# facebookresearch/hyperreel

Hardware: NVIDIA H100
Metric: Mrays/s at 65k-ray x 32-sample batch (higher is better)
Workload: dtype f32 (sample net bf16x3 split on wgmma, fp32 accumulate)

## Files before the change

hyperreel_b200/csrc/hr_mlp_tc2.cu:

```cuda
#include <cuda.h>
#include <cuda_bf16.h>

#include <cstdio>
#include <cstdlib>
#include <cstring>

#include "hr_encode.cuh"
#include "hr_handle.h"
#include "hr_tc_prims.cuh"

namespace hr {

namespace tc2 {
using namespace tc;

constexpr int NSTAGE = 4;
constexpr int STAGE_BYTES = 8192;
constexpr int KSTEP_BYTES = 4096;
constexpr int CONSUMERS = 2;
constexpr int NTHREADS = (CONSUMERS + 1) * 128;
constexpr int PRODUCER_REGS = 40;
constexpr int CONSUMER_REGS = 232;
static_assert(128 * PRODUCER_REGS + CONSUMERS * 128 * CONSUMER_REGS <= 65536, "register file");

constexpr int A_BYTES = 16 * KSTEP_BYTES;
constexpr int OFF_AHI = 0;
constexpr int OFF_ALO = OFF_AHI + A_BYTES;
constexpr int X_BYTES = 4 * KSTEP_BYTES;
constexpr int OFF_X = OFF_ALO + A_BYTES;
constexpr int OFF_B = OFF_X + 2 * X_BYTES;
constexpr int OFF_BAR = OFF_B + CONSUMERS * NSTAGE * STAGE_BYTES;
constexpr int SMEM_BYTES = OFF_BAR + 128;
static_assert(SMEM_BYTES <= 232448, "shared memory budget");

constexpr int BAR_FULL = 0;
constexpr int BAR_EMPTY = BAR_FULL + CONSUMERS * NSTAGE;
static_assert((BAR_EMPTY + CONSUMERS * NSTAGE) * 8 <= 128, "barrier block");

constexpr int NB_RET = 3;
constexpr int NB_WR = 5;
constexpr int NB_XW = 7;
constexpr int NB_XR = 9;

}

template <int W, bool SAVE, bool NARROW>
__global__ void __launch_bounds__(tc2::NTHREADS, 1)
mlp_tc2_kernel(const __grid_constant__ hr_config cfg, const __grid_constant__ MlpTcPack pk, const float* __restrict__ rays,
               float* __restrict__ heads, long long n_rays, float* __restrict__ rays_copy, const TrainSave sv) {
  using namespace tc2;
  constexpr int WH = W / 2;
  constexpr int NACC = WH / 2;
  constexpr int NK = W / 16;
  constexpr int NKH = NK / 2;
  constexpr int IMG_BYTES = WH * 64;
  constexpr int KPS = STAGE_BYTES / IMG_BYTES;
  static_assert(KPS * IMG_BYTES == STAGE_BYTES && NKH % KPS == 0 && NK * KSTEP_BYTES <= A_BYTES, "pass width");
  extern __shared__ __align__(128) uint8_t smem[];
  const uint32_t sbase = smem_u32(smem);
  const int tid = threadIdx.x, warp = tid >> 5, lane = tid & 31;
  auto bar = [&](int slot) -> uint32_t { return sbase + OFF_BAR + slot * 8; };

  {
    const char* w = reinterpret_cast<const char*>(pk.wpack);
    const long long lines = pk.wpack_bytes >> 7;
    for (long long i = (long long)blockIdx.x * NTHREADS + tid; i < lines; i += (long long)gridDim.x * NTHREADS)
      asm volatile("prefetch.global.L2 [%0];" ::"l"(w + i * 128));
  }
  for (int i = tid; i < (2 * X_BYTES) / 16; i += NTHREADS)
    reinterpret_cast<uint4*>(smem + OFF_X)[i] = make_uint4(0u, 0u, 0u, 0u);
  if (tid == 0) {
    for (int s = 0; s < CONSUMERS * NSTAGE; ++s) { mbar_init(bar(BAR_FULL + s), 1); mbar_init(bar(BAR_EMPTY + s), 1); }
    asm volatile("fence.mbarrier_init.release.cluster;" ::: "memory");
  }
  __syncthreads();

  const long long n_tiles = (n_rays + BM - 1) / BM;
  const int n_passes = pk.n_passes;
  const long long n_iters = ((long long)blockIdx.x < n_tiles) ? (n_tiles - 1 - blockIdx.x) / gridDim.x + 1 : 0;

  if (warp >= CONSUMERS * 4) {
    setmaxnreg_dec<PRODUCER_REGS>();
    const int g = warp - CONSUMERS * 4;
    if (g < CONSUMERS && lane == 0) {
      const long long half_bytes = pk.wpack_bytes / CONSUMERS;
      const int n_stages = (int)(half_bytes / STAGE_BYTES);
      const uint32_t full0 = bar(BAR_FULL + g * NSTAGE), empty0 = bar(BAR_EMPTY + g * NSTAGE);
      const uint32_t ring = sbase + OFF_B + (uint32_t)(g * NSTAGE * STAGE_BYTES);
      uint32_t stage = 0, phase = 0;
      for (long long iter = 0; iter < n_iters; ++iter) {
        const uint8_t* src = reinterpret_cast<const uint8_t*>(pk.wpack) + g * half_bytes;
        for (int i = 0; i < n_stages; ++i) {
          mbar_wait(empty0 + stage * 8, phase ^ 1);
          mbar_expect_tx(full0 + stage * 8, STAGE_BYTES);
          bulk_g2s(ring + stage * STAGE_BYTES, src, STAGE_BYTES, full0 + stage * 8);
          src += STAGE_BYTES;
          if (++stage == NSTAGE) { stage = 0; phase ^= 1; }
        }
      }
    }
    return;
  }

  setmaxnreg_inc<CONSUMER_REGS>();
  const int wg = warp >> 2;
  const int wt = tid & 127;
  const int rowq = (warp & 3) * 16 + (lane >> 2);
  const int q2 = (lane & 3) * 2;
  const int col0 = wg * WH;
  const int in_chunks = pk.in_chunks;
  const int L = cfg.mlp_layers;
  const uint32_t x_lo_off = (uint32_t)(2 * in_chunks * KSTEP_BYTES);
  const uint32_t full0 = bar(BAR_FULL + wg * NSTAGE), empty0 = bar(BAR_EMPTY + wg * NSTAGE);
  const uint32_t ring = sbase + OFF_B + (uint32_t)(wg * NSTAGE * STAGE_BYTES);
  const bool vec_ok = ((reinterpret_cast<uintptr_t>(rays) | reinterpret_cast<uintptr_t>(rays_copy)) & 15) == 0;
  int x_last = 0;
  for (int p = 0; p < n_passes; ++p)
    if (pk.passes[p].first_chunk == 0) x_last = p;
  uint32_t stage = 0, phase = 0;
  int pend = -1;

  float acc[2][NACC];

  auto stage_begin = [&]() {
    mbar_wait(full0 + stage * 8, phase);
    wgmma_fence();
    acc_fence(acc[0]);
    acc_fence(acc[1]);
  };
  auto stage_end = [&]() {
    wgmma_commit();
    acc_fence(acc[0]);
    acc_fence(acc[1]);
    wgmma_wait<1>();
    if (pend >= 0 && wt == 0) mbar_arrive(empty0 + pend * 8);
    pend = (int)stage;
    if (++stage == NSTAGE) { stage = 0; phase ^= 1; }
  };
  auto b_img = [&](int sub) -> uint32_t { return ring + stage * STAGE_BYTES + (uint32_t)sub * IMG_BYTES; };
  auto kstep = [&](uint32_t a, uint32_t a_lo, uint32_t b, uint32_t scale) {
    const uint64_t bh = gmma_desc(b, WH * 16, 128), bl = gmma_desc(b + WH * 32, WH * 16, 128);
    const uint64_t ah0 = gmma_desc(a, 2048, 128), ah1 = gmma_desc(a + 1024, 2048, 128);
    const uint64_t al0 = gmma_desc(a + a_lo, 2048, 128), al1 = gmma_desc(a + a_lo + 1024, 2048, 128);
    wgmma_ss(acc[0], ah0, bh, scale);
    wgmma_ss(acc[1], ah1, bh, scale);
    wgmma_ss(acc[0], al0, bh, 1u);
    wgmma_ss(acc[1], al1, bh, 1u);
    wgmma_ss(acc[0], ah0, bl, 1u);
    wgmma_ss(acc[1], ah1, bl, 1u);
  };
  auto run_pass = [&](const TcPass& P, bool fresh, bool x_ret, bool ret) {
    int ki = 0;
    if (P.first_chunk == 0) {
      for (; ki < 2 * in_chunks; ki += KPS) {
        stage_begin();
#pragma unroll
        for (int sub = 0; sub < KPS; ++sub)
          kstep(sbase + OFF_X + (uint32_t)(ki + sub) * KSTEP_BYTES, x_lo_off, b_img(sub), (ki + sub) != 0 ? 1u : 0u);
        stage_end();
      }
    }
    if (P.first_chunk + P.n_chunks > in_chunks) {
      const uint32_t scale0 = ki != 0 ? 1u : 0u;
#pragma unroll
      for (int kk = 0; kk < NK; ++kk) {
        if (kk % KPS == 0) {
          if (fresh && kk == (wg == 0 ? NKH : 0)) {
            if (wg == 0) pair_arrive(NB_WR + 0);
            pair_wait(NB_WR + (wg ^ 1));
          }
          stage_begin();
        }
        kstep(sbase + OFF_AHI + (uint32_t)kk * KSTEP_BYTES, OFF_ALO - OFF_AHI, b_img(kk % KPS), kk != 0 ? 1u : scale0);
        if (kk % KPS == KPS - 1) {
          stage_end();
          if (x_ret && kk == KPS - 1) pair_arrive(NB_XR + wg);
          if (ret && wg == 1 && kk == NKH + KPS - 1) pair_arrive(NB_RET + 1);
        }
      }
    }
  };
  auto drain = [&]() {
    wgmma_wait<0>();
    acc_fence(acc[0]);
    acc_fence(acc[1]);
    if (pend >= 0 && wt == 0) mbar_arrive(empty0 + pend * 8);
    pend = -1;
  };
  const int st_row = (warp & 3) * 16 + 8 * ((lane >> 3) & 1) + (lane & 7);
  const uint32_t st_off = ks_slot(st_row, lane >> 4);
  auto store_hidden = [&](const float* bias, int layer, long long tile) {
#pragma unroll
    for (int kk = 0; kk < NKH; ++kk) {
      float2 b[2];
#pragma unroll
      for (int jj = 0; jj < 2; ++jj) b[jj] = __ldg(reinterpret_cast<const float2*>(bias + col0 + 8 * (2 * kk + jj) + q2));
#pragma unroll
      for (int m = 0; m < 2; ++m) {
        uint32_t hi[4], lo[4];
#pragma unroll
        for (int jj = 0; jj < 2; ++jj) {
          const int j = 2 * kk + jj, k = col0 + 8 * j + q2;
#pragma unroll
          for (int h = 0; h < 2; ++h) {
            float t0 = acc[m][4 * j + 2 * h] + b[jj].x, t1 = acc[m][4 * j + 2 * h + 1] + b[jj].y;
            t0 = fmaxf(t0, t0 * cfg.leaky_slope);
            t1 = fmaxf(t1, t1 * cfg.leaky_slope);
            split2(t0, t1, hi[2 * jj + h], lo[2 * jj + h]);
            if constexpr (SAVE) {
              const long long ray = tile * BM + 64 * m + rowq + 8 * h;
              if (ray < n_rays) *reinterpret_cast<float2*>(sv.act + layer * sv.act_stride + ray * W + k) = make_float2(t0, t1);
            }
          }
        }
        const uint32_t a = sbase + st_off + (uint32_t)m * 1024u + (uint32_t)(wg * NKH + kk) * KSTEP_BYTES;
        stmatrix_x4(a + OFF_AHI, hi);
        stmatrix_x4(a + OFF_ALO, lo);
      }
    }
  };
  auto encode = [&](long long tile, bool after_x) {
    if (after_x) pair_wait(NB_XR + (wg ^ 1));
    const int r = wg * 64 + (wt & 63), part = wt >> 6;
    const long long ray = tile * BM + r;
    auto put = [&](int k, float val) {
      if constexpr (SAVE) {
        if (ray < n_rays) sv.enc[ray * sv.ld_enc + k] = val;
      }
      const __nv_bfloat16 hi = __float2bfloat16_rn(val);
      const __nv_bfloat16 lo = __float2bfloat16_rn(val - __bfloat162float(hi));
      const uint32_t off = (uint32_t)(k >> 4) * KSTEP_BYTES + ks_slot(r, (k >> 3) & 1) + (uint32_t)(k & 7) * 2u;
      *reinterpret_cast<__nv_bfloat16*>(smem + OFF_X + off) = hi;
      *reinterpret_cast<__nv_bfloat16*>(smem + OFF_X + x_lo_off + off) = lo;
    };
    if (ray < n_rays) {
      float rbuf[16];
      const float* src = rays + ray * cfg.c_in;
      if (cfg.c_in == 8 && vec_ok) {
        const float4 a = *reinterpret_cast<const float4*>(src), b = *reinterpret_cast<const float4*>(src + 4);
        rbuf[0] = a.x; rbuf[1] = a.y; rbuf[2] = a.z; rbuf[3] = a.w; rbuf[4] = b.x; rbuf[5] = b.y; rbuf[6] = b.z; rbuf[7] = b.w;
        if (rays_copy != nullptr && part == 0) {
          float4* dst = reinterpret_cast<float4*>(rays_copy + ray * 8);
          dst[0] = a; dst[1] = b;
        }
      } else {
        for (int i = 0; i < cfg.c_in; ++i) rbuf[i] = src[i];
        if (rays_copy != nullptr && part == 0)
          for (int i = 0; i < cfg.c_in; ++i) rays_copy[ray * cfg.c_in + i] = rbuf[i];
      }
      encode_ray_features(cfg, rbuf, part, 2, put);
      if constexpr (SAVE) {
        if (part == 0)
          for (int k = cfg.mlp_in; k < sv.ld_enc; ++k) sv.enc[ray * sv.ld_enc + k] = 0.0f;
      }
    } else if (part == 0) {
      for (int k = 0; k < cfg.mlp_in; ++k) put(k, 0.0f);
    }
    fence_async_smem();
    wg_sync(1 + wg);
    pair_arrive(NB_XW + wg);
  };

  for (long long iter = 0; iter < n_iters; ++iter) {
    const long long tile = iter * gridDim.x + blockIdx.x;
    const bool more = iter + 1 < n_iters;
    if (iter == 0) encode(tile, false);
    pair_wait(NB_XW + (wg ^ 1));
    for (int p = 0; p < n_passes; ++p) {
      const TcPass& P = pk.passes[p];
      const bool reads_a = P.first_chunk + P.n_chunks > in_chunks;
      const bool hidden = p < L - 1;
      const bool ret = reads_a && (hidden || (p == n_passes - 1 && more));
      const bool x_ret = p == x_last && more;
      run_pass(P, reads_a && P.wait_a != 0, x_ret, ret);
      drain();
      if (x_ret && !reads_a) pair_arrive(NB_XR + wg);
      if (ret && wg == 0) pair_arrive(NB_RET + 0);
      if (hidden) {
        wg_sync(1 + wg);
        if (p > 0 || iter > 0) pair_wait(NB_RET + (wg ^ 1));
        store_hidden(pk.bias + P.bias_off, p, tile);
        fence_async_smem();
        wg_sync(1 + wg);
        if (wg == 1) pair_arrive(NB_WR + 1);
      } else {
        const float* bias = pk.bias + P.bias_off;
        if constexpr (SAVE) {
#pragma unroll
          for (int m = 0; m < 2; ++m)
#pragma unroll
            for (int h = 0; h < 2; ++h) {
              const long long ray = tile * BM + 64 * m + rowq + 8 * h;
              if (ray >= n_rays) continue;
              float* row = heads + ray * cfg.mlp_out;
#pragma unroll
              for (int j = 0; j < WH / 8; ++j) {
                const int c = col0 + 8 * j + q2;
                if (P.out_col0 + c < cfg.mlp_out) {
                  const float2 b = __ldg(reinterpret_cast<const float2*>(bias + c));
                  const int c0 = P.out_col0 + c, c1 = c0 + 1, S = cfg.n_samples;
                  row[(c0 % S) * cfg.head_stride + c0 / S] = acc[m][4 * j + 2 * h] + b.x;
                  if (c1 < cfg.mlp_out) row[(c1 % S) * cfg.head_stride + c1 / S] = acc[m][4 * j + 2 * h + 1] + b.y;
                }
              }
            }
        } else if constexpr (NARROW) {
          const bool pairs = (cfg.mlp_out % 2) == 0 && (reinterpret_cast<uintptr_t>(heads) & 7) == 0;
#pragma unroll
          for (int j = 0; j < WH / 8; ++j) {
            const int c = col0 + 8 * j + q2, c0 = P.out_col0 + c;
            const float2 b = __ldg(reinterpret_cast<const float2*>(bias + c));
#pragma unroll
            for (int m = 0; m < 2; ++m)
#pragma unroll
              for (int h = 0; h < 2; ++h) {
                const long long ray = tile * BM + 64 * m + rowq + 8 * h;
                if (ray >= n_rays || c0 >= cfg.mlp_out) continue;
                float* dst = heads + ray * cfg.mlp_out + c0;
                const float v0 = acc[m][4 * j + 2 * h] + b.x, v1 = acc[m][4 * j + 2 * h + 1] + b.y;
                if (pairs) {
                  *reinterpret_cast<float2*>(dst) = make_float2(v0, v1);
                } else {
                  dst[0] = v0;
                  if (c0 + 1 < cfg.mlp_out) dst[1] = v1;
                }
              }
          }
        } else {
          const bool odd = (lane & 1) != 0;
#pragma unroll
          for (int jp = 0; jp < WH / 16; ++jp) {
            const int j = 2 * jp, c = col0 + 8 * j + q2;
            const float2 b0 = __ldg(reinterpret_cast<const float2*>(bias + c));
            const float2 b1 = __ldg(reinterpret_cast<const float2*>(bias + c + 8));
#pragma unroll
            for (int m = 0; m < 2; ++m)
#pragma unroll
              for (int h = 0; h < 2; ++h) {
                const float2 v0 = make_float2(acc[m][4 * j + 2 * h] + b0.x, acc[m][4 * j + 2 * h + 1] + b0.y);
                const float2 v1 = make_float2(acc[m][4 * j + 4 + 2 * h] + b1.x, acc[m][4 * j + 4 + 2 * h + 1] + b1.y);
                const float2 send = odd ? v0 : v1;
                const float2 recv = make_float2(__shfl_xor_sync(0xffffffffu, send.x, 1), __shfl_xor_sync(0xffffffffu, send.y, 1));
                const int c4 = odd ? c + 6 : c;
                const long long ray = tile * BM + 64 * m + rowq + 8 * h;
                if (ray < n_rays && P.out_col0 + c4 < cfg.mlp_out)
                  *reinterpret_cast<float4*>(heads + ray * cfg.mlp_out + P.out_col0 + c4) =
                      odd ? make_float4(recv.x, recv.y, v1.x, v1.y) : make_float4(v0.x, v0.y, recv.x, recv.y);
              }
          }
        }
      }
      if (x_ret) encode(tile + gridDim.x, true);
    }
  }
}

int pack_mlp_tc2(SampleNet& net, const float* const* w_dev, const float* const* b_dev, cudaStream_t st) {
  const hr_config& c = net.cfg;
  MlpTcPack& pk = net.tc;
  size_t& alloc_bytes = net.tc_alloc_bytes;
  int& alloc_bias = net.tc_alloc_bias;
  const int W = c.mlp_width;
  if (W != 128 && W != 256) return hr_fail("tensor-core sample net: hidden width must be 128 or 256 (got %d)", W);
  if (c.mlp_in > 64) return hr_fail("tensor-core sample net: encoded input wider than 64 features (%d)", c.mlp_in);
  const int in_chunks = (c.mlp_in + 31) / 32;
  const int L = c.mlp_layers;
  MlpTcPack np_{};
  np_.in_chunks = in_chunks;
  int np = 0, bias_off = 0;
  size_t bytes = 0;
  for (int l = 0; l < L; ++l) {
    const bool last = (l == L - 1);
    const int out = last ? c.mlp_out : W;
    const int n_parts = (out + W - 1) / W;
    for (int part = 0; part < n_parts; ++part) {
      if (np >= HR_TC_MAX_PASSES) return hr_fail("tensor-core sample net: too many passes (%d output columns)", c.mlp_out);
      TcPass& P = np_.passes[np++];
      const bool reads_input = (l == 0 || l == c.mlp_skip);
      P.layer = l;
      P.n = W;
      P.first_chunk = reads_input ? 0 : in_chunks;
      P.n_chunks = (l == 0) ? in_chunks : (W / 32 + (reads_input ? in_chunks : 0));
      P.bias_off = bias_off;
      P.is_final = last ? 1 : 0;
      P.out_col0 = part * W;
      P.wait_a = (part == 0) ? 1 : 0;
      bias_off += P.n;
      bytes += (size_t)P.n_chunks * 2 * P.n * 64;
    }
  }
  np_.n_passes = np;
  np_.bias_count = bias_off;
  np_.wpack_bytes = (long long)bytes;
  if (alloc_bytes != bytes || alloc_bias != bias_off || !pk.wpack) {
    if (pk.wpack) cudaFree(const_cast<void*>(pk.wpack));
    if (pk.bias) cudaFree(const_cast<float*>(pk.bias));
    pk.wpack = nullptr; pk.bias = nullptr;
    alloc_bytes = 0; alloc_bias = 0;
    void* wp = nullptr; float* bp = nullptr;
    cudaError_t e = cudaMalloc(&wp, bytes);
    if (e != cudaSuccess) return hr_fail("cudaMalloc(tc weights %zu): %s", bytes, cudaGetErrorString(e));
    e = cudaMalloc((void**)&bp, (size_t)bias_off * sizeof(float));
    if (e != cudaSuccess) { cudaFree(wp); return hr_fail("cudaMalloc(tc bias): %s", cudaGetErrorString(e)); }
    np_.wpack = wp; np_.bias = bp;
    alloc_bytes = bytes; alloc_bias = bias_off;
    for (int narrow = 0; narrow < 2 && e == cudaSuccess; ++narrow) {
      auto kern = (W == 256) ? (narrow ? mlp_tc2_kernel<256, false, true> : mlp_tc2_kernel<256, false, false>)
                             : (narrow ? mlp_tc2_kernel<128, false, true> : mlp_tc2_kernel<128, false, false>);
      e = cudaFuncSetAttribute(kern, cudaFuncAttributeMaxDynamicSharedMemorySize, tc2::SMEM_BYTES);
    }
    if (e != cudaSuccess) return hr_fail("cudaFuncSetAttribute(mlp_tc2_kernel): %s", cudaGetErrorString(e));
  } else {
    np_.wpack = pk.wpack; np_.bias = pk.bias;
  }
  pk = np_;
  uint8_t* wp = (uint8_t*)const_cast<void*>(pk.wpack);
  float* bp = const_cast<float*>(pk.bias);
  const int WH = W / 2;
  for (int half = 0; half < 2; ++half) {
    size_t off = (size_t)half * (bytes / 2);
    for (int p = 0; p < np; ++p) {
      const TcPass& P = pk.passes[p];
      const int l = P.layer;
      const bool last = (l == L - 1), skip = (l == c.mlp_skip), first = (l == 0);
      const int in_src = first ? c.mlp_in : (skip ? c.mlp_in + W : W);
      launch_pack_tc_pass(w_dev[l], b_dev[l], wp + off, bp + P.bias_off + half * WH, WH, P.first_chunk, P.n_chunks, in_src,
                          c.mlp_in, skip ? 1 : 0, in_chunks, last ? c.mlp_out : W, last ? c.n_samples : 0, c.head_stride,
                          P.out_col0 + half * WH, st);
      off += (size_t)P.n_chunks * 2 * WH * 64;
    }
  }
  cudaError_t e = cudaGetLastError();
  if (e != cudaSuccess) return hr_fail("tc pack launch failed: %s", cudaGetErrorString(e));
  return 0;
}

void free_mlp_tc2(SampleNet& net) {
  if (net.tc.wpack) cudaFree(const_cast<void*>(net.tc.wpack));
  if (net.tc.bias) cudaFree(const_cast<float*>(net.tc.bias));
  net.tc.wpack = nullptr; net.tc.bias = nullptr;
  net.tc_alloc_bytes = 0; net.tc_alloc_bias = 0;
}

cudaError_t launch_mlp_tc2(const hr_config& cfg, const MlpTcPack& pk, const float* rays, float* heads, long long n, int num_sms,
                           cudaStream_t stream, float* rays_copy) {
  long long tiles = (n + tc::BM - 1) / tc::BM;
  int grid = (int)(tiles < num_sms ? tiles : num_sms);
  if (grid < 1) grid = 1;
  const bool narrow = (cfg.mlp_out % 4) != 0 || ((uintptr_t)heads % 16) != 0;
  auto kern = cfg.mlp_width == 256 ? (narrow ? mlp_tc2_kernel<256, false, true> : mlp_tc2_kernel<256, false, false>)
                                   : (narrow ? mlp_tc2_kernel<128, false, true> : mlp_tc2_kernel<128, false, false>);
  if (cfg.mlp_width != 256 && cfg.mlp_width != 128) return cudaErrorInvalidValue;
  kern<<<grid, tc2::NTHREADS, tc2::SMEM_BYTES, stream>>>(cfg, pk, rays, heads, n, rays_copy, TrainSave{});
  return cudaGetLastError();
}

cudaError_t launch_mlp_tc2_train(const hr_config& cfg, const MlpTcPack& pk, const float* rays, float* heads, long long n,
                                 int num_sms, cudaStream_t stream, const TrainSave& sv) {
  long long tiles = (n + tc::BM - 1) / tc::BM;
  int grid = (int)(tiles < num_sms ? tiles : num_sms);
  if (grid < 1) grid = 1;
  auto kern = cfg.mlp_width == 256 ? mlp_tc2_kernel<256, true, false> : mlp_tc2_kernel<128, true, false>;
  if (cfg.mlp_width != 256 && cfg.mlp_width != 128) return cudaErrorInvalidValue;
  cudaError_t e = cudaFuncSetAttribute(kern, cudaFuncAttributeMaxDynamicSharedMemorySize, tc2::SMEM_BYTES);
  if (e != cudaSuccess) return e;
  kern<<<grid, tc2::NTHREADS, tc2::SMEM_BYTES, stream>>>(cfg, pk, rays, heads, n, nullptr, sv);
  return cudaGetLastError();
}

}
```

Baseline: 156.9.

## Move next-tile ray encoding to producer-warpgroup encoder warps with mbarrier handoff

Encoding of the next tile's input features moves off the consumer warpgroups and onto the two idle warps of the producer warpgroup. These warps fill the X buffer, which is double-buffered when the input fits in one chunk, and hand it over through full/empty mbarriers. This replaces the named-barrier handshake and the inline encode that consumers ran after each tile. Consumer registers drop from 232 to 224 to give the producer warpgroup 56, which risks spills in the consumer accumulator path, and only 64 threads now encode each tile.

```diff
diff --git a/hyperreel_b200/csrc/hr_mlp_tc2.cu b/hyperreel_b200/csrc/hr_mlp_tc2.cu
--- a/hyperreel_b200/csrc/hr_mlp_tc2.cu
+++ b/hyperreel_b200/csrc/hr_mlp_tc2.cu
@@ -19,28 +19,31 @@
 constexpr int KSTEP_BYTES = 4096;
 constexpr int CONSUMERS = 2;
 constexpr int NTHREADS = (CONSUMERS + 1) * 128;
-constexpr int PRODUCER_REGS = 40;
-constexpr int CONSUMER_REGS = 232;
+constexpr int ENC_THREADS = 64;
+constexpr int PRODUCER_REGS = 56;
+constexpr int CONSUMER_REGS = 224;
 static_assert(128 * PRODUCER_REGS + CONSUMERS * 128 * CONSUMER_REGS <= 65536, "register file");
 
 constexpr int A_BYTES = 16 * KSTEP_BYTES;
 constexpr int OFF_AHI = 0;
 constexpr int OFF_ALO = OFF_AHI + A_BYTES;
-constexpr int X_BYTES = 4 * KSTEP_BYTES;
+constexpr int X_CHUNK_BYTES = 4 * KSTEP_BYTES;
 constexpr int OFF_X = OFF_ALO + A_BYTES;
-constexpr int OFF_B = OFF_X + 2 * X_BYTES;
+constexpr int OFF_B = OFF_X + 2 * X_CHUNK_BYTES;
 constexpr int OFF_BAR = OFF_B + CONSUMERS * NSTAGE * STAGE_BYTES;
-constexpr int SMEM_BYTES = OFF_BAR + 128;
+constexpr int BAR_BYTES = 160;
+constexpr int SMEM_BYTES = OFF_BAR + BAR_BYTES;
 static_assert(SMEM_BYTES <= 232448, "shared memory budget");
 
 constexpr int BAR_FULL = 0;
 constexpr int BAR_EMPTY = BAR_FULL + CONSUMERS * NSTAGE;
-static_assert((BAR_EMPTY + CONSUMERS * NSTAGE) * 8 <= 128, "barrier block");
+constexpr int BAR_X_FULL = BAR_EMPTY + CONSUMERS * NSTAGE;
+constexpr int BAR_X_EMPTY = BAR_X_FULL + 2;
+static_assert((BAR_X_EMPTY + 2) * 8 <= BAR_BYTES, "barrier block");
 
 constexpr int NB_RET = 3;
 constexpr int NB_WR = 5;
-constexpr int NB_XW = 7;
-constexpr int NB_XR = 9;
+constexpr int NB_X0 = 7;
 
 }
 
@@ -67,10 +70,11 @@
     for (long long i = (long long)blockIdx.x * NTHREADS + tid; i < lines; i += (long long)gridDim.x * NTHREADS)
       asm volatile("prefetch.global.L2 [%0];" ::"l"(w + i * 128));
   }
-  for (int i = tid; i < (2 * X_BYTES) / 16; i += NTHREADS)
+  for (int i = tid; i < (2 * X_CHUNK_BYTES) / 16; i += NTHREADS)
     reinterpret_cast<uint4*>(smem + OFF_X)[i] = make_uint4(0u, 0u, 0u, 0u);
   if (tid == 0) {
     for (int s = 0; s < CONSUMERS * NSTAGE; ++s) { mbar_init(bar(BAR_FULL + s), 1); mbar_init(bar(BAR_EMPTY + s), 1); }
+    for (int s = 0; s < 2; ++s) { mbar_init(bar(BAR_X_FULL + s), ENC_THREADS); mbar_init(bar(BAR_X_EMPTY + s), CONSUMERS); }
     asm volatile("fence.mbarrier_init.release.cluster;" ::: "memory");
   }
   __syncthreads();
@@ -78,6 +82,54 @@
   const long long n_tiles = (n_rays + BM - 1) / BM;
   const int n_passes = pk.n_passes;
   const long long n_iters = ((long long)blockIdx.x < n_tiles) ? (n_tiles - 1 - blockIdx.x) / gridDim.x + 1 : 0;
+  const int in_chunks = pk.in_chunks;
+  const int x_slots = in_chunks == 1 ? 2 : 1;
+  const uint32_t x_slot_bytes = (uint32_t)(in_chunks * X_CHUNK_BYTES);
+  const uint32_t x_lo_off = (uint32_t)(2 * in_chunks * KSTEP_BYTES);
+  const bool vec_ok = cfg.c_in == 8 && ((reinterpret_cast<uintptr_t>(rays) | reinterpret_cast<uintptr_t>(rays_copy)) & 15) == 0;
+  auto load_row = [&](long long tile, int r, float* rbuf) {
+    const long long ray = tile * BM + r;
+    if (ray >= n_rays) return;
+    const float* src = rays + ray * cfg.c_in;
+    if (vec_ok) {
+      const float4 a = *reinterpret_cast<const float4*>(src), b = *reinterpret_cast<const float4*>(src + 4);
+      rbuf[0] = a.x; rbuf[1] = a.y; rbuf[2] = a.z; rbuf[3] = a.w; rbuf[4] = b.x; rbuf[5] = b.y; rbuf[6] = b.z; rbuf[7] = b.w;
+    } else {
+      for (int i = 0; i < cfg.c_in; ++i) rbuf[i] = src[i];
+    }
+  };
+  auto encode_row = [&](long long tile, int r, int part, int nparts, const float* rbuf, int slot) {
+    const long long ray = tile * BM + r;
+    uint8_t* xs = smem + OFF_X + slot * x_slot_bytes;
+    auto put = [&](int k, float val) {
+      if constexpr (SAVE) {
+        if (ray < n_rays) sv.enc[ray * sv.ld_enc + k] = val;
+      }
+      const __nv_bfloat16 hi = __float2bfloat16_rn(val);
+      const __nv_bfloat16 lo = __float2bfloat16_rn(val - __bfloat162float(hi));
+      const uint32_t off = (uint32_t)(k >> 4) * KSTEP_BYTES + ks_slot(r, (k >> 3) & 1) + (uint32_t)(k & 7) * 2u;
+      *reinterpret_cast<__nv_bfloat16*>(xs + off) = hi;
+      *reinterpret_cast<__nv_bfloat16*>(xs + x_lo_off + off) = lo;
+    };
+    if (ray < n_rays) {
+      if (rays_copy != nullptr && part == 0) {
+        if (vec_ok) {
+          float4* dst = reinterpret_cast<float4*>(rays_copy + ray * 8);
+          dst[0] = make_float4(rbuf[0], rbuf[1], rbuf[2], rbuf[3]);
+          dst[1] = make_float4(rbuf[4], rbuf[5], rbuf[6], rbuf[7]);
+        } else {
+          for (int i = 0; i < cfg.c_in; ++i) rays_copy[ray * cfg.c_in + i] = rbuf[i];
+        }
+      }
+      encode_ray_features(cfg, rbuf, part, nparts, put);
+      if constexpr (SAVE) {
+        if (part == 0)
+          for (int k = cfg.mlp_in; k < sv.ld_enc; ++k) sv.enc[ray * sv.ld_enc + k] = 0.0f;
+      }
+    } else if (part == 0) {
+      for (int k = 0; k < cfg.mlp_in; ++k) put(k, 0.0f);
+    }
+  };
 
   if (warp >= CONSUMERS * 4) {
     setmaxnreg_dec<PRODUCER_REGS>();
@@ -98,6 +150,20 @@
           if (++stage == NSTAGE) { stage = 0; phase ^= 1; }
         }
       }
+    } else if (g >= CONSUMERS) {
+      const int et = tid - (CONSUMERS * 4 + CONSUMERS) * 32;
+      for (long long iter = 1; iter < n_iters; ++iter) {
+        const long long tile = iter * gridDim.x + blockIdx.x;
+        const int slot = (int)(iter % x_slots);
+        float rbuf[2][16];
+#pragma unroll
+        for (int j = 0; j < 2; ++j) load_row(tile, j * ENC_THREADS + et, rbuf[j]);
+        mbar_wait(bar(BAR_X_EMPTY + slot), ((uint32_t)(iter / x_slots) & 1u) ^ 1u);
+#pragma unroll
+        for (int j = 0; j < 2; ++j) encode_row(tile, j * ENC_THREADS + et, 0, 1, rbuf[j], slot);
+        fence_async_smem();
+        mbar_arrive(bar(BAR_X_FULL + slot));
+      }
     }
     return;
   }
@@ -108,12 +174,9 @@
   const int rowq = (warp & 3) * 16 + (lane >> 2);
   const int q2 = (lane & 3) * 2;
   const int col0 = wg * WH;
-  const int in_chunks = pk.in_chunks;
   const int L = cfg.mlp_layers;
-  const uint32_t x_lo_off = (uint32_t)(2 * in_chunks * KSTEP_BYTES);
   const uint32_t full0 = bar(BAR_FULL + wg * NSTAGE), empty0 = bar(BAR_EMPTY + wg * NSTAGE);
   const uint32_t ring = sbase + OFF_B + (uint32_t)(wg * NSTAGE * STAGE_BYTES);
-  const bool vec_ok = ((reinterpret_cast<uintptr_t>(rays) | reinterpret_cast<uintptr_t>(rays_copy)) & 15) == 0;
   int x_last = 0;
   for (int p = 0; p < n_passes; ++p)
     if (pk.passes[p].first_chunk == 0) x_last = p;
@@ -149,14 +212,14 @@
     wgmma_ss(acc[0], ah0, bl, 1u);
     wgmma_ss(acc[1], ah1, bl, 1u);
   };
-  auto run_pass = [&](const TcPass& P, bool fresh, bool x_ret, bool ret) {
+  auto run_pass = [&](const TcPass& P, uint32_t x, uint32_t x_empty, bool fresh, bool x_ret, bool ret) {
     int ki = 0;
     if (P.first_chunk == 0) {
       for (; ki < 2 * in_chunks; ki += KPS) {
         stage_begin();
 #pragma unroll
         for (int sub = 0; sub < KPS; ++sub)
-          kstep(sbase + OFF_X + (uint32_t)(ki + sub) * KSTEP_BYTES, x_lo_off, b_img(sub), (ki + sub) != 0 ? 1u : 0u);
+          kstep(x + (uint32_t)(ki + sub) * KSTEP_BYTES, x_lo_off, b_img(sub), (ki + sub) != 0 ? 1u : 0u);
         stage_end();
       }
     }
@@ -174,7 +237,7 @@
         kstep(sbase + OFF_AHI + (uint32_t)kk * KSTEP_BYTES, OFF_ALO - OFF_AHI, b_img(kk % KPS), kk != 0 ? 1u : scale0);
         if (kk % KPS == KPS - 1) {
           stage_end();
-          if (x_ret && kk == KPS - 1) pair_arrive(NB_XR + wg);
+          if (x_ret && kk == KPS - 1 && wt == 0) mbar_arrive(x_empty);
           if (ret && wg == 1 && kk == NKH + KPS - 1) pair_arrive(NB_RET + 1);
         }
       }
@@ -219,62 +282,30 @@
       }
     }
   };
-  auto encode = [&](long long tile, bool after_x) {
-    if (after_x) pair_wait(NB_XR + (wg ^ 1));
-    const int r = wg * 64 + (wt & 63), part = wt >> 6;
-    const long long ray = tile * BM + r;
-    auto put = [&](int k, float val) {
-      if constexpr (SAVE) {
-        if (ray < n_rays) sv.enc[ray * sv.ld_enc + k] = val;
-      }
-      const __nv_bfloat16 hi = __float2bfloat16_rn(val);
-      const __nv_bfloat16 lo = __float2bfloat16_rn(val - __bfloat162float(hi));
-      const uint32_t off = (uint32_t)(k >> 4) * KSTEP_BYTES + ks_slot(r, (k >> 3) & 1) + (uint32_t)(k & 7) * 2u;
-      *reinterpret_cast<__nv_bfloat16*>(smem + OFF_X + off) = hi;
-      *reinterpret_cast<__nv_bfloat16*>(smem + OFF_X + x_lo_off + off) = lo;
-    };
-    if (ray < n_rays) {
-      float rbuf[16];
-      const float* src = rays + ray * cfg.c_in;
-      if (cfg.c_in == 8 && vec_ok) {
-        const float4 a = *reinterpret_cast<const float4*>(src), b = *reinterpret_cast<const float4*>(src + 4);
-        rbuf[0] = a.x; rbuf[1] = a.y; rbuf[2] = a.z; rbuf[3] = a.w; rbuf[4] = b.x; rbuf[5] = b.y; rbuf[6] = b.z; rbuf[7] = b.w;
-        if (rays_copy != nullptr && part == 0) {
-          float4* dst = reinterpret_cast<float4*>(rays_copy + ray * 8);
-          dst[0] = a; dst[1] = b;
-        }
-      } else {
-        for (int i = 0; i < cfg.c_in; ++i) rbuf[i] = src[i];
-        if (rays_copy != nullptr && part == 0)
-          for (int i = 0; i < cfg.c_in; ++i) rays_copy[ray * cfg.c_in + i] = rbuf[i];
-      }
-      encode_ray_features(cfg, rbuf, part, 2, put);
-      if constexpr (SAVE) {
-        if (part == 0)
-          for (int k = cfg.mlp_in; k < sv.ld_enc; ++k) sv.enc[ray * sv.ld_enc + k] = 0.0f;
-      }
-    } else if (part == 0) {
-      for (int k = 0; k < cfg.mlp_in; ++k) put(k, 0.0f);
-    }
-    fence_async_smem();
-    wg_sync(1 + wg);
-    pair_arrive(NB_XW + wg);
-  };
-
   for (long long iter = 0; iter < n_iters; ++iter) {
     const long long tile = iter * gridDim.x + blockIdx.x;
     const bool more = iter + 1 < n_iters;
-    if (iter == 0) encode(tile, false);
-    pair_wait(NB_XW + (wg ^ 1));
+    const int slot = (int)(iter % x_slots);
+    const uint32_t x = sbase + OFF_X + slot * x_slot_bytes, x_empty = bar(BAR_X_EMPTY + slot);
+    if (iter == 0) {
+      float rbuf[16];
+      const int r = wg * 64 + (wt & 63), part = wt >> 6;
+      load_row(tile, r, rbuf);
+      encode_row(tile, r, part, 2, rbuf, slot);
+      fence_async_smem();
+      pair_wait(NB_X0);
+    } else {
+      mbar_wait(bar(BAR_X_FULL + slot), (uint32_t)((iter - 1) / x_slots) & 1u);
+    }
     for (int p = 0; p < n_passes; ++p) {
       const TcPass& P = pk.passes[p];
       const bool reads_a = P.first_chunk + P.n_chunks > in_chunks;
       const bool hidden = p < L - 1;
       const bool ret = reads_a && (hidden || (p == n_passes - 1 && more));
-      const bool x_ret = p == x_last && more;
-      run_pass(P, reads_a && P.wait_a != 0, x_ret, ret);
+      const bool x_ret = p == x_last;
+      run_pass(P, x, x_empty, reads_a && P.wait_a != 0, x_ret, ret);
       drain();
-      if (x_ret && !reads_a) pair_arrive(NB_XR + wg);
+      if (x_ret && !reads_a && wt == 0) mbar_arrive(x_empty);
       if (ret && wg == 0) pair_arrive(NB_RET + 0);
       if (hidden) {
         wg_sync(1 + wg);
@@ -350,7 +381,6 @@
           }
         }
       }
-      if (x_ret) encode(tile + gridDim.x, true);
     }
   }
 }
```

Result: no change. 157.2 (median of 6 runs) (+0.2%).
